# 14chanwa/remotesensingProject

Measured on AMD Instinct MI355X. Metric: Mpixel*disparity-hypotheses/s, higher is better.
Workload: dtype f32

## Files before the change

remotesensingproject_amd/build.py:

```python
from __future__ import annotations

import os
import re
import subprocess
import sys

HERE = os.path.dirname(os.path.abspath(__file__))
CSRC = os.path.join(HERE, "csrc")
OBJ = os.path.join(CSRC, "build")
SO = os.path.join(CSRC, "librslf_hip.so")
INCLUDE = os.path.join(os.path.dirname(HERE), "include")
COMMON = ["rslf_internal.hpp", "rslf_plan.hpp", "rslf_scratch.hpp", "rslf_device.hpp", "k2_taps.hpp", os.path.join(INCLUDE, "rslf_hip.h")]
UNITS = {
    "rslf_core.hip": ["k0_pack.hpp"],
    "rslf_pile.hip": ["k1_edge.hpp", "k_compact.hpp", "k2_scan.hpp", "k2_reg.hpp", "k2_stream.hpp", "k3_median.hpp"],
    "rslf_chip_a.hip": ["k2_scan.hpp", "k2_chip.hpp"],
    "rslf_chip_b.hip": ["k2_scan.hpp", "k2_chip.hpp"],
    "rslf_chip_c.hip": ["k2_scan.hpp", "k2_chip.hpp"],
    "rslf_scores.hip": ["k2_scan.hpp", "k2_reg.hpp", "k2_scores.hpp"],
    "rslf_peaks.hip": ["k8_peaks.hpp", "k8_peak_rule.hpp", "rslf_plan_peaks.hpp"],
    "rslf_subgrid.hip": ["k2_scan.hpp", "k9_subgrid.hpp", "k8_peak_rule.hpp", "rslf_plan_subgrid.hpp"],
    "rslf_sweep.hip": ["k3_median.hpp", "k4_propagate.hpp", "k_compact.hpp", "k2_scan.hpp", "k7_line_conf.hpp", "rslf_plan_subgrid.hpp",
                       "rslf_plan_sweep_peaks.hpp", "rslf_plan_peaks.hpp", "rslf_plan_sweep_gate.hpp", "k11_f2c_peak_rule.hpp"],
    "rslf_sweep_peaks.hip": ["k2_scan.hpp", "k10_sweep_peaks.hpp", "k10_peak_merge.hpp", "k8_peak_rule.hpp", "rslf_plan_sweep_peaks.hpp",
                             "rslf_plan_peaks.hpp", "rslf_plan_subgrid.hpp"],
    "rslf_f2c.hip": ["k5_f2c.hpp", "rslf_plan_f2c_peaks.hpp", "rslf_plan_peaks.hpp", "rslf_plan_f2c_consistency.hpp",
                     "rslf_plan_consistency.hpp", "k12_consistency_rule.hpp", "rslf_plan_derivative.hpp", "k17_derivative_rule.hpp"],
    "rslf_f2c_keep.hip": ["rslf_plan_f2c_peaks.hpp", "rslf_plan_peaks.hpp", "rslf_plan_sweep_gate.hpp", "k11_f2c_peak_rule.hpp",
                          "rslf_plan_f2c_consistency.hpp", "rslf_plan_consistency.hpp", "k12_consistency_rule.hpp"],
    "rslf_f2c_peaks.hip": ["k11_f2c_peaks.hpp", "k11_f2c_peak_rule.hpp", "rslf_plan_f2c_peaks.hpp", "rslf_plan_peaks.hpp"],
    "rslf_render.hip": ["k6_render.hpp", "rslf_plan_render.hpp"],
    "rslf_consistency.hip": ["k12_consistency.hpp", "k12_consistency_rule.hpp", "rslf_plan_consistency.hpp", "k13_f2c_consistency.hpp",
                             "rslf_plan_f2c_consistency.hpp"],
    "rslf_warp.hip": ["k14_view_warp.hpp", "k14_warp_rule.hpp", "rslf_plan_warp.hpp", "k12_consistency_rule.hpp"],
    "rslf_novel.hip": ["k15_novel_view.hpp", "k15_novel_rule.hpp", "rslf_plan_novel.hpp", "k14_warp_rule.hpp", "rslf_plan_warp.hpp",
                       "k12_consistency_rule.hpp"],
    "rslf_dilate.hip": ["k16_dilate.hpp", "k16_dilate_rule.hpp", "rslf_plan_dilate.hpp"],
    "rslf_derivative.hip": ["k17_derivative.hpp", "k17_derivative_rule.hpp", "rslf_plan_derivative.hpp"],
    "rslf_multi.hip": [],
    "rslf_multi_sweep.hip": [],
}
SOURCES = list(UNITS)

HIPCC_FLAGS = [
    "--offload-arch=gfx950",
# ... 131 lines not shown
```

remotesensingproject_amd/csrc/k2_reg.hpp:

```cpp
#pragma once

#include "k2_scan.hpp"
#include "k2_taps.hpp"

namespace rslf {

#ifndef RSLF_REG_GB104
#define RSLF_REG_GB104 8
#endif
constexpr int gather_batch(int c) { return c == 1 ? 8 : 4; }
constexpr int kPadSlack = 16;

template <int SPAD, int C, bool PK, bool KONLY>
__device__ __forceinline__ void mean_shift_pass(const float (&R)[PK ? 1 : C][PK ? 1 : SPAD], const f2 (&R2)[PK ? C : 1][PK ? SPAD / 2 : 1],
                                                int S, float kq, const float (&rbar)[C], float (&A)[C], float& B)
{
    static_assert(!KONLY || (C == 1 && !PK), "the K-only pass is written for the scalar one-channel blocks");
    if constexpr (PK) {
        f2 rb2[C];
        const f2 kq2 = {kq, kq};
#pragma unroll
        for (int c = 0; c < C; c++)
            rb2[c] = f2{rbar[c], rbar[c]};
        constexpr int kBlk = (C == 1) ? 8 : 4;
#pragma unroll
        for (int s0 = 0; s0 < SPAD; s0 += kBlk) {
            if (!(s0 < SPAD - kPadSlack || s0 < S))
                continue;
            if constexpr (C == 1) {
                f2 P[4], K[4];
                const f2 r4[4] = {R2[0][s0 / 2], R2[0][s0 / 2 + 1], R2[0][s0 / 2 + 2], R2[0][s0 / 2 + 3]};
                mean_shift_pk_octet(r4, rb2[0], kq2, P, K);
#pragma unroll
                for (int j = 0; j < 4; j++) {
                    A[0] = A[0] + P[j].x;
                    B = B + K[j].x;
                    A[0] = A[0] + P[j].y;
                    B = B + K[j].y;
                }
            } else {
                f2 Pa[3], Pb[3], Ka, Kb;
                const f2 ra[3] = {R2[0][s0 / 2], R2[1][s0 / 2], R2[C - 1][s0 / 2]};
                const f2 rb[3] = {R2[0][s0 / 2 + 1], R2[1][s0 / 2 + 1], R2[C - 1][s0 / 2 + 1]};
                const f2 m[3] = {rb2[0], rb2[C > 1 ? 1 : 0], rb2[C - 1]};
                mean_shift_pk_rgb_quad(ra, rb, m, kq2, Pa, Pb, Ka, Kb);
#pragma unroll
                for (int c = 0; c < C; c++)
                    A[c] = A[c] + Pa[c].x;
                B = B + Ka.x;
#pragma unroll
                for (int c = 0; c < C; c++)
                    A[c] = A[c] + Pa[c].y;
                B = B + Ka.y;
#pragma unroll
                for (int c = 0; c < C; c++)
                    A[c] = A[c] + Pb[c].x;
                B = B + Kb.x;
#pragma unroll
                for (int c = 0; c < C; c++)
                    A[c] = A[c] + Pb[c].y;
                B = B + Kb.y;
            }
        }
    } else if (C == 1) {
#pragma unroll
        for (int s0 = 0; s0 < SPAD; s0 += 4) {
            if (s0 + 4 <= SPAD - kPadSlack || s0 + 4 <= S) {
                if constexpr (KONLY)
                    mean_shift_group4_k(R[0][s0], R[0][s0 + 1], R[0][s0 + 2], R[0][s0 + 3], rbar[0], kq, B);
                else
                    mean_shift_group4(R[0][s0], R[0][s0 + 1], R[0][s0 + 2], R[0][s0 + 3], rbar[0], kq, A[0], B);
            } else {
#pragma unroll
                for (int j = 0; j < 3; j++)
                    if (s0 + j < S) {
                        if constexpr (KONLY)
                            mean_shift_group1_k(R[0][s0 + j], rbar[0], kq, B);
                        else
                            mean_shift_group1(R[0][s0 + j], rbar[0], kq, A[0], B);
                    }
            }
        }
    } else {
#pragma unroll
        for (int s = 0; s < SPAD; s++) {
            if (!(s < SPAD - kPadSlack || s < S))
                continue;
            float q[C];
#pragma unroll
            for (int c = 0; c < C; c++) {
                const float delta = R[c][s] - rbar[c];
                const float tq = kq * delta;
                q[c] = tq * delta;
            }
            float qs = q[0];
            if (C == 3) {
                qs = q[0] + q[C - 1];
                qs = qs + q[C > 1 ? 1 : 0];
            }
            const float K = kernel_weight(qs);
#pragma unroll
            for (int c = 0; c < C; c++) {
                const float pr = R[c][s] * K;
                A[c] = A[c] + pr;
            }
            B = B + K;
        }
    }
}

template <int SPAD, int C, int BATCH>
__device__ __forceinline__ void tap_table_batch(const float* epi, const float* otab, const int* tboff, const f2* tw, unsigned du_bytes,
                                                float uf, int S, int stride_s, bool from_table, int g, int& rowoff, float (&R)[C][SPAD])
{
// ... 27 lines not shown
    }
    rowoff += BATCH * stride_s;
#pragma unroll
    for (int j = 0; j < BATCH; j++) {
        const int s = g * BATCH + j;
#pragma unroll
        for (int c = 0; c < C; c++) {
            e0[c][j] = kSentinel;
            e1[c][j] = 0.0f;
        }
        if (s < SPAD - kPadSlack || s < S) {
            const float* p = (const float*)((const char*)epi + bo[j]);
#pragma unroll
            for (int c = 0; c < C; c++) {
                e0[c][j] = p[c];
                e1[c][j] = p[C + c];
            }
        }
    }
#pragma unroll
    for (int j = 0; j < BATCH; j++) {
        const int s = g * BATCH + j;
#pragma unroll
        for (int c = 0; c < C; c++) {
            const float m0 = om[j] * e0[c][j];
            const float m1 = tt[j] * e1[c][j];
            const float r = m0 + m1;
            R[c][s] = (s < SPAD - kPadSlack || s < S) ? r : kSentinel;
        }
    }
}

template <int SPAD, int C, bool BORDER, bool UNIFORM_D, bool PK, int GB = 0, class BestT = Best<C>, bool LANE_D = false,
          bool TRIM = false, bool TAPS = false>
__device__ __forceinline__ void scan_reg_body(const ScanArgs& a, int v, int u, int d0, int d1, BestT& best,
                                              float* __restrict__ otab, int dlane = 0, int dstep = 1)
{
    static_assert(!LANE_D || !UNIFORM_D, "hypotheses in the lanes: every lane has its own view offsets");
    constexpr int kGatherBatch = GB > 0 ? GB : (C == 1 && !PK && SPAD == 104 && RSLF_REG_GB104 == 13) ? 13 : gather_batch(C);
    static_assert(SPAD % kGatherBatch == 0 && (!PK || kGatherBatch % 2 == 0), "whole batches, whole pairs");
    static_assert(SPAD % 8 == 0, "slot counts are multiples of 8");
    static_assert(!TAPS || (UNIFORM_D && !BORDER && !PK), "the tap table belongs to the interior scalar uniform-D row form");
    const VolView& vol = a.vol;
    const float* epi = vol.row(v, 0);
    const float uf = (float)u;
    const int Um1 = vol.U - 1;
    const unsigned Um1_bits = __float_as_uint((float)Um1);
    const int S = vol.S;
    const int lane = threadIdx.x & 63;
    const long long o = (long long)v * vol.U + u;
    const float dmin = a.dmin_vu ? a.dmin_vu[o] : a.dmin;
    const float dmax = a.dmax_vu ? a.dmax_vu[o] : a.dmax;
    const float range = dmax - dmin;
    const float denom = (float)(a.dim_d - 1);
    const float kq = (C == 1) ? a.k.k1 : a.k.inv_h2;
    const float slope = a.k.slope;
    const int stride_s = (int)vol.stride_s;
    float centre[C];
#pragma unroll
    for (int c = 0; c < C; c++)
        centre[c] = epi[(long long)a.s_hat * vol.stride_s + u * C + c];
    int* const tboff = TAPS ? reinterpret_cast<int*>(otab + SPAD) : nullptr;
    f2* const tw = TAPS ? reinterpret_cast<f2*>(otab + 2 * SPAD) : nullptr;
    int u_first = 0, u_last = 0;
    unsigned du_bytes = 0;
    bool taps_on = false;
    if constexpr (TAPS) {
        u_first = __builtin_amdgcn_readfirstlane(u);
        u_last = __builtin_amdgcn_readlane(u, 63);
        const int du = u - u_first;
        du_bytes = (unsigned)(du * C) << 2;
        taps_on = a.tap_table != 0 && __all(du == min(lane, u_last - u_first));
    }

#pragma unroll 1
    for (int dk = d0; dk < d1; dk += (LANE_D ? dstep : 1)) {
        const int d = LANE_D ? min(dk + dlane, d1 - 1) : dk;
        const float Dd = hypothesis(dmin, range, denom, d);
        float R[PK ? 1 : C][PK ? 1 : SPAD];
        f2 R2[PK ? C : 1][PK ? SPAD / 2 : 1];
        int card = BORDER ? 0 : S;
        float Ss0 = (float)a.s_hat;
        asm volatile("" : "+v"(Ss0));
        int rowoff = 0;
        asm volatile("" : "+s"(rowoff));
        unsigned fastb = 0;
        if (UNIFORM_D) {
            int lane_s = lane, tile_first = u_first, tile_last = u_last;
            if constexpr (TAPS)
                asm volatile("" : "+v"(lane_s), "+s"(tile_first), "+s"(tile_last));
#pragma unroll
            for (int s0 = 0; s0 < SPAD; s0 += 64) {
                const int s = s0 + lane_s;
                float off = (float)(a.s_hat - s) * Dd;
                off = off * slope;
                if (SPAD % 64 == 0 || s < SPAD)
                    otab[s] = off;
                if constexpr (TAPS) {
                    if (taps_on) {
                        const TapEntry e = tap_entry(off, tile_first, tile_last, vol.U, C, __mul24(s, stride_s));
                        if (SPAD % 64 == 0 || s < SPAD) {
                            tboff[s] = e.byteoff;
                            tw[s] = f2{e.t, e.omt};
                        }
                        unsigned long long m = __ballot(e.fast);
                        m &= m >> 1;
                        m &= m >> 2;
                        m &= m >> 4;
                        static_assert(!TAPS || kGatherBatch == 8, "the batch bits are gathered for batches of eight samples");
#pragma unroll
                        for (int k = 0; k < 8; k++)
                            if (s0 + 8 * k < SPAD)
                                fastb |= ((unsigned)(m >> (8 * k)) & 1u) << (s0 / 8 + k);
                    }
                }
            }
            __builtin_amdgcn_wave_barrier();
            if constexpr (TAPS)
                fastb = __builtin_amdgcn_readfirstlane(fastb & (S >= SPAD ? ~0u : (1u << (S / kGatherBatch)) - 1u));
        }
#pragma unroll
        for (int g = 0; g < SPAD / kGatherBatch; g++) {
            if constexpr (TAPS) {
                tap_table_batch<SPAD, C, kGatherBatch>(epi, otab, tboff, tw, du_bytes, uf, S, stride_s, (fastb >> g) & 1u, g, rowoff, R);
            } else {
                float tt[kGatherBatch], e0[C][kGatherBatch], e1[C][kGatherBatch];
                bool ok[kGatherBatch];
#pragma unroll
                for (int j = 0; j < kGatherBatch; j++) {
                    const int s = g * kGatherBatch + j;
                    tt[j] = 0.0f;
                    ok[j] = false;
#pragma unroll
                    for (int c = 0; c < C; c++) {
                        e0[c][j] = kSentinel;
                        e1[c][j] = 0.0f;
                    }
                    if (s < SPAD - kPadSlack || s < S) {
                        float x;
                        if (UNIFORM_D) {
                            x = otab[s];
                        } else {
                            x = (Ss0 - (float)s) * Dd;
                            x = x * slope;
                        }
                        x = x + uf;
                        tt[j] = lerp_weight(x);
                        int i0 = floor_to_int(x);
                        ok[j] = true;
                        if (BORDER) {
                            ok[j] = __float_as_uint(x) <= Um1_bits;
                            i0 = ok[j] ? i0 : 0;
                        }
                        const unsigned byteoff = (unsigned)(i0 * C + rowoff) << 2;
                        const float* p = (const float*)((const char*)epi + byteoff);
// ... 22 lines not shown
                        if constexpr (PK) {
                            if (s & 1)
                                R2[c][s >> 1].y = val;
                            else
                                R2[c][s >> 1].x = val;
                        } else {
                            R[c][s] = val;
                        }
                    }
                    if (BORDER)
                        card += ok[j] ? 1 : 0;
                }
            }
            {
                const int b = g * kGatherBatch;
#pragma unroll
                for (int c = 0; c < C; c++) {
                    if constexpr (PK) {
                        asm volatile("" : "+v"(R2[c][b / 2]), "+v"(R2[c][b / 2 + 1]));
                        if (kGatherBatch == 8)
                            asm volatile("" : "+v"(R2[c][b / 2 + 2]), "+v"(R2[c][b / 2 + 3]));
                        static_assert(!PK || kGatherBatch == 4 || kGatherBatch == 8, "pair pinning is written for 4 and 8");
                    } else if (kGatherBatch != 4 && kGatherBatch != 8) {
#pragma unroll
                        for (int j = 0; j < kGatherBatch; j++)
                            asm volatile("" : "+v"(R[c][b + j]));
                    } else {
                        asm volatile("" : "+v"(R[c][b + 0]), "+v"(R[c][b + 1]), "+v"(R[c][b + 2]), "+v"(R[c][b + 3]));
                        if (kGatherBatch == 8)
                            asm volatile("" : "+v"(R[c][b + kGatherBatch - 4]), "+v"(R[c][b + kGatherBatch - 3]),
                                              "+v"(R[c][b + kGatherBatch - 2]), "+v"(R[c][b + kGatherBatch - 1]));
                    }
                }
                if (BORDER)
                    asm volatile("" : "+s"(rowoff), "+v"(Ss0), "+v"(card));
                else
                    asm volatile("" : "+s"(rowoff), "+v"(Ss0));
            }
        }

        float rbar[C];
#pragma unroll
        for (int c = 0; c < C; c++)
            rbar[c] = centre[c];
        float B = 0.0f;
#pragma unroll 1
        for (int it = 0; it < a.k.n_iter; it++) {
            float A[C];
#pragma unroll
            for (int c = 0; c < C; c++)
                A[c] = 0.0f;
            B = 0.0f;
            if constexpr (TRIM) {
                if (it == a.k.n_iter - 1) {
                    mean_shift_pass<SPAD, C, PK, true>(R, R2, S, kq, rbar, A, B);
                    break;
                }
            }
            mean_shift_pass<SPAD, C, PK, false>(R, R2, S, kq, rbar, A, B);
#pragma unroll
            for (int c = 0; c < C; c++) {
                const float qd = (B != 0.0f) ? (A[c] / B) : 0.0f;
                rbar[c] = (qd > 0.0f) ? qd : 0.0f;
            }
        }
        const float cardf = (float)card;
        float sc = (card != 0) ? (B / cardf) : 0.0f;
        sc = (sc > 0.0f) ? sc : 0.0f;
        if (!LANE_D || dk + dlane < d1)
            best.offer(sc, d, Dd, rbar);
    }
}

template <int C>
struct LastPassRbar {
    __device__ __forceinline__ void operator()(const ScanArgs& a, long long o, float Dd, float (&rbar)[C]) const
    {
        if (a.k.n_iter == 0)
            return;
        const VolView& vol = a.vol;
        const int v = (int)(o / vol.U);
        const int u = (int)(o - (long long)v * vol.U);
        const float* epi = vol.row(v, 0);
        const float uf = (float)u;
        const unsigned Um1_bits = __float_as_uint((float)(vol.U - 1));
        const float kq = (C == 1) ? a.k.k1 : a.k.inv_h2;
        const float Ss0 = (float)a.s_hat;
        const int S = vol.S;
        float A[C];
#pragma unroll
        for (int c = 0; c < C; c++)
            A[c] = 0.0f;
// ... 156 lines not shown
                const float m0 = w[j].y * e0[j];
                const float m1 = w[j].x * e1[j];
                R[0][g * BATCH + j] = m0 + m1;
            }
#pragma unroll
            for (int j = 0; j < BATCH; j++)
                asm volatile("" : "+v"(R[0][g * BATCH + j]));
#pragma unroll
            for (int j = 0; j < BATCH; j++)
                cur[j] = nxt[j];
        }

        float rbar[C] = {centre};
        float B = 0.0f;
#pragma unroll 1
        for (int it = 0; it < a.k.n_iter; it++) {
            float A[C] = {0.0f};
            B = 0.0f;
            if (it == a.k.n_iter - 1) {
                mean_shift_pass<SPAD, C, false, true>(R, R2, S, kq, rbar, A, B);
                break;
            }
            mean_shift_pass<SPAD, C, false, false>(R, R2, S, kq, rbar, A, B);
            const float qd = (B != 0.0f) ? (A[0] / B) : 0.0f;
            rbar[0] = (qd > 0.0f) ? qd : 0.0f;
        }
        const float cardf = (float)S;
        float sc = (S != 0) ? (B / cardf) : 0.0f;
        sc = (sc > 0.0f) ? sc : 0.0f;
        best.offer(sc, d, Dd, rbar);
    }
}

template <int SPAD, int C>
using ScanRegRbarFix = std::conditional_t<scan_reg_trim(SPAD, C), LastPassRbar<C>, NoRbarFix>;

template <int SPAD, int C, class BestT>
__device__ __forceinline__ void scan_reg_rows(const ScanArgs& a, int v, int u, int d0, int d1, BestT& best, float* otab)
{
    constexpr bool PK = scan_reg_packed_math(SPAD, C);
    constexpr bool kTaps = scan_reg_tap_table(SPAD, C);
    if (a.dmin_vu) {
        scan_reg_body<SPAD, C, true, false, PK, 0, BestT, false, scan_reg_trim(SPAD, C)>(a, v, u, d0, d1, best, otab);
        return;
    }
    const float max_ds = (float)max(a.s_hat, a.vol.S - 1 - a.s_hat);
    const float range = a.dmax - a.dmin, denom = (float)(a.dim_d - 1);
    const float uf = (float)u, Um1 = (float)(a.vol.U - 1);
    if constexpr (scan_reg_scalar_taps(SPAD, C)) {
        typedef const __attribute__((address_space(4))) float* FloatPtr;
        typedef const __attribute__((address_space(4))) int* IntPtr;
        const bool rx = a.rx_off != nullptr;
        auto form = [&](int d) -> int {
            const float Dd = rx ? ((FloatPtr)a.rx_D)[d] : hypothesis(a.dmin, range, denom, d);
            const float reach = max_ds * fabsf(Dd) * fabsf(a.k.slope) + 2.0f;
            const bool in = __all((uf - reach >= 0.0f) && (uf + reach <= Um1));
            return !in ? 0 : (rx && ((IntPtr)a.rx_exact)[d]) ? 2 : 1;
        };
        int d = d0;
        while (d < d1) {
            const int f = form(d);
            int e = d + 1;
            while (e < d1 && form(e) == f)
                e++;
            if (f == 2)
                scan_reg_body_scalar<SPAD>(a, v, u, d, e, best);
            else if (f == 1)
                scan_reg_body<SPAD, C, false, true, PK, 0, BestT, false, scan_reg_trim(SPAD, C), kTaps>(a, v, u, d, e, best, otab);
            else
                scan_reg_body<SPAD, C, true, true, PK, 0, BestT, false, scan_reg_trim(SPAD, C)>(a, v, u, d, e, best, otab);
            d = e;
        }
        return;
    }
    auto interior = [&](int d) -> bool {
        const float reach = max_ds * fabsf(hypothesis(a.dmin, range, denom, d)) * fabsf(a.k.slope) + 2.0f;
        return __all((uf - reach >= 0.0f) && (uf + reach <= Um1));
    };
    int d = d0;
    while (d < d1) {
        const bool in = interior(d);
        int e = d + 1;
        while (e < d1 && interior(e) == in)
            e++;
        if (in)
            scan_reg_body<SPAD, C, false, true, PK, 0, BestT, false, scan_reg_trim(SPAD, C), kTaps>(a, v, u, d, e, best, otab);
        else
            scan_reg_body<SPAD, C, true, true, PK, 0, BestT, false, scan_reg_trim(SPAD, C)>(a, v, u, d, e, best, otab);
        d = e;
    }
}

template <int SPAD, int C>
__global__ __launch_bounds__(64 * kScanWaves) __attribute__((amdgpu_waves_per_eu(scan_reg_waves(SPAD, C), scan_reg_waves(SPAD, C))))
void k2_scan_reg(ScanArgs a)
{
    __shared__ __attribute__((aligned(16))) float s_otab[kScanWaves][SPAD * (scan_reg_tap_table(SPAD, C) ? 4 : 1)];
    float* otab = s_otab[__builtin_amdgcn_readfirstlane(threadIdx.x >> 6)];
    constexpr bool kEpiDyn = false;
    float* const epi_lds = nullptr;
    const int epi_stride = 0;
    using Fix = ScanRegRbarFix<SPAD, C>;
    if constexpr (scan_reg_best_in_lds(SPAD, C)) {
        __shared__ float s_best[kScanWaves][BestLds<C>::kFloats];
        BestLds<C> running(s_best[__builtin_amdgcn_readfirstlane(threadIdx.x >> 6)]);
        RSLF_SCAN_ROW_TILE_FIX((running.init(), scan_reg_rows<SPAD, C>(a, v, u, d0, d1, running, otab), running.load(best)), Fix{})
    } else {
        RSLF_SCAN_ROW_TILE_FIX((scan_reg_rows<SPAD, C>(a, v, u, d0, d1, best, otab)), Fix{})
    }
}

#ifndef RSLF_PACKED_LONG_GB
#define RSLF_PACKED_LONG_GB 4
#endif
constexpr bool packed_long_unit(int spad, int c) { return c == 1 && spad >= 80 && spad <= 128 && spad % RSLF_PACKED_LONG_GB == 0; }
constexpr int packed_waves(int spad, int c) { return packed_long_unit(spad, c) ? 2 : scan_reg_waves(spad + 24, c); }
constexpr int packed_gather_batch(int spad, int c) { return packed_long_unit(spad, c) ? spad / RSLF_PACKED_LONG_GB : 0; }

template <int SPAD, int C>
__global__ __launch_bounds__(64 * kScanWaves) __attribute__((amdgpu_waves_per_eu(packed_waves(SPAD, C), packed_waves(SPAD, C))))
void k2_scan_reg_packed(ScanArgs a)
// ... 48 lines not shown
```

remotesensingproject_amd/csrc/k2_scan.hpp:

```cpp
#pragma once

#include <type_traits>

#include "rslf_device.hpp"

namespace rslf {

constexpr int kScanWaves = 4;
#ifndef RSLF_XCD_ROW_INTERLEAVE
#define RSLF_XCD_ROW_INTERLEAVE 1
#endif

struct ScanArgs {
    VolView vol;
    const int* list;
    const int* count;
    const float* dmin_vu;
    const float* dmax_vu;
    float dmin, dmax;
    int dim_d, s_hat;
    ScanConsts k;
    float* Ce;
    uint8_t* Ce_mask;
    float* Cd;
    float* depth;
    float* rbar;
    int32_t* idx;
    float* score;
    int tile_w;
    int tiles_per_row;
    int logical_blocks;
    int per_xcd;
    int groups;
    struct Partial* partial;
    int* ticket;
    int v0;
    int packed;
    const int* packed_n;
    int packed_adapt;
    int stream_park;
    int stream_wave_floats;
    float stream_frac_max;
    int px_waves;
    const int* rowbase;
    int row_min;
    int tap_table;
    const long long* rx_off;
    const float* rx_w;
    const float* rx_D;
    const int* rx_exact;
};


struct Partial {
    float score, D;
    int d;
    float rbar[3];
    double sum;
};

template <int C>
struct Best {
    float score;
    int d;
    float D;
    float rbar[C];
    double sum;
    __device__ __forceinline__ void init()
    {
        score = -1.0f;
        d = 0;
        D = 0.0f;
#pragma unroll
        for (int c = 0; c < C; c++)
            rbar[c] = 0.0f;
        sum = 0.0;
    }
    __device__ __forceinline__ void offer(float sc, int dd, float Dd, const float (&rb)[C])
    {
// ... 545 lines not shown
```

remotesensingproject_amd/csrc/k2_scores.hpp:

```cpp
#pragma once

#include "k2_reg.hpp"
#include "rslf_plan.hpp"

namespace rslf {

constexpr int kScoreRun = plan::kScoreRun;
constexpr int kScorePitch = kScoreRun + 1;
static_assert(64 % kScoreRun == 0, "a store instruction covers whole runs");

struct ScoreDst {
    float* scores;
    int v_first;
};

template <int C>
struct ScoreRows {
    float* park;
    const int* pix;
    float* row;
    int dim_d, d_lo, d_hi;
    __device__ __forceinline__ ScoreRows(float* park_, int* pix_, const ScanArgs& a, const ScoreDst& dst, int v, int u, bool active,
                                         int d0, int d1)
        : park(park_), pix(pix_), row(dst.scores + (size_t)(v - dst.v_first) * (size_t)a.vol.U * (size_t)a.dim_d), dim_d(a.dim_d),
// ... 6 lines not shown
        const int k = (d - d_lo) % kScoreRun;
        park[(threadIdx.x & 63) * kScorePitch + k] = sc;
        if (k == kScoreRun - 1 || d == d_hi - 1)
            flush(d - k, k + 1);
    }
    __device__ __forceinline__ void flush(int d_first, int n)
    {
        __builtin_amdgcn_fence(__ATOMIC_RELEASE, "wavefront");
        __builtin_amdgcn_wave_barrier();
        const int lane = threadIdx.x & 63;
        const int j = lane % kScoreRun, q = lane / kScoreRun;
#pragma unroll 4
        for (int p0 = 0; p0 < 64; p0 += 64 / kScoreRun) {
            const int p = p0 + q;
            const float sc = park[p * kScorePitch + j];
            const int u = pix[p];
            if (j < n && u >= 0)
                row[(size_t)u * (size_t)dim_d + (size_t)(d_first + j)] = sc;
        }
        __builtin_amdgcn_wave_barrier();
        __builtin_amdgcn_fence(__ATOMIC_ACQUIRE, "wavefront");
    }
};

constexpr bool score_rows_trim(int spad, int c) { return c == 1 && !scan_reg_packed_math(spad, c); }
constexpr bool score_rows_tap_table(int spad, int c) { return scan_reg_tap_table(spad, c) && score_rows_trim(spad, c); }

template <int SPAD, int C>
__device__ __forceinline__ void score_reg_rows(const ScanArgs& a, int v, int u, int d0, int d1, ScoreRows<C>& rows, float* otab)
{
    constexpr bool PK = scan_reg_packed_math(SPAD, C);
    constexpr bool kTrim = score_rows_trim(SPAD, C);
    constexpr bool kTaps = score_rows_tap_table(SPAD, C);
    if (a.dmin_vu) {
        scan_reg_body<SPAD, C, true, false, PK, 0, ScoreRows<C>, false, kTrim>(a, v, u, d0, d1, rows, otab);
        return;
    }
    const float max_ds = (float)max(a.s_hat, a.vol.S - 1 - a.s_hat);
    const float range = a.dmax - a.dmin, denom = (float)(a.dim_d - 1);
    const float uf = (float)u, Um1 = (float)(a.vol.U - 1);
    auto interior = [&](int d) -> bool {
        const float reach = max_ds * fabsf(hypothesis(a.dmin, range, denom, d)) * fabsf(a.k.slope) + 2.0f;
        return __all((uf - reach >= 0.0f) && (uf + reach <= Um1));
    };
    int d = d0;
    while (d < d1) {
        const bool in = interior(d);
        int e = d + 1;
        while (e < d1 && interior(e) == in)
            e++;
        if (in)
            scan_reg_body<SPAD, C, false, true, PK, 0, ScoreRows<C>, false, kTrim, kTaps>(a, v, u, d, e, rows, otab);
        else
            scan_reg_body<SPAD, C, true, true, PK, 0, ScoreRows<C>, false, kTrim>(a, v, u, d, e, rows, otab);
        d = e;
    }
}

#define RSLF_SCORE_ROW_TILE(SCAN_CALL)                                                                                     \
    __shared__ float s_park[kScanWaves][64 * kScorePitch];                                                                 \
    __shared__ int s_pix[kScanWaves][64];                                                                                  \
    int v, u, d0, d1;                                                                                                      \
    bool active;                                                                                                           \
    const int lb = RSLF_XCD_ROW_INTERLEAVE ? xcd_logical_block_rows(blockIdx.x, a.tiles_per_row * a.groups)                \
                                           : xcd_logical_block(blockIdx.x, a.per_xcd);                                     \
    if (!scan_tile(a, lb, v, u, active))                                                                                   \
        return;                                                                                                            \
    scan_chunk(a, lb % a.groups, d0, d1);                                                                                  \
    const int wave = __builtin_amdgcn_readfirstlane(threadIdx.x >> 6);                                                     \
    ScoreRows<C> rows(s_park[wave], s_pix[wave], a, dst, v, u, active, d0, d1);                                            \
    SCAN_CALL;

template <int SPAD, int C>
__global__ __launch_bounds__(64 * kScanWaves) __attribute__((amdgpu_waves_per_eu(scan_reg_waves(SPAD, C), scan_reg_waves(SPAD, C))))
void k2_score_rows_reg(ScanArgs a, ScoreDst dst)
{
    constexpr int kTable = score_rows_tap_table(SPAD, C) ? 4 : 1;
    __shared__ __attribute__((aligned(16))) float s_otab[kScanWaves][SPAD * kTable];
    static_assert(sizeof(float) * kScanWaves * (64 * kScorePitch + 64 + SPAD * kTable) == plan::score_lds_bytes(SPAD, kTable) &&
                      plan::score_lds_bytes(SPAD, kTable) <= plan::kScoreLdsLimit, "rslf_plan.hpp states this kernel's LDS");
    float* otab = s_otab[__builtin_amdgcn_readfirstlane(threadIdx.x >> 6)];
    RSLF_SCORE_ROW_TILE((score_reg_rows<SPAD, C>(a, v, u, d0, d1, rows, otab)))
}

template <int C>
__global__ __launch_bounds__(64 * kScanWaves) void k2_score_rows_generic(ScanArgs a, ScoreDst dst)
{
// ... 44 lines not shown
```

remotesensingproject_amd/csrc/rslf_core.hip:

```cpp
#include "rslf_internal.hpp"

#include <algorithm>
#include <cmath>

#include "k0_pack.hpp"

using namespace rslf;


namespace rslf {

char* last_error_buffer()
{
    static thread_local char g_err[512] = "";
    return g_err;
}

static std::atomic<int> g_inject[kInjectSites];

bool inject_hit(InjectSite site)
{
    std::atomic<int>& c = g_inject[site];
    int v = c.load(std::memory_order_relaxed);
    while (v > 0)
// ... 186 lines not shown
    return RSLF_OK;
}
RSLF_API_CATCH

extern "C" int rslf_ctx_set_stream(rslf_ctx* ctx, void* hip_stream) RSLF_API_TRY
{
    if (!ctx)
        return fail(RSLF_ERR_INVALID_ARG, "ctx is NULL");
    ctx->stream = (hipStream_t)hip_stream;
    return RSLF_OK;
}
RSLF_API_CATCH

extern "C" int rslf_ctx_set_debug(rslf_ctx* ctx, const char* key, int value) RSLF_API_TRY
{
    if (!ctx || !key)
        return fail(RSLF_ERR_INVALID_ARG, "ctx/key is NULL");
    if (strcmp(key, "force_scan") == 0 && value >= 0 && value <= 2)
        ctx->force_scan = value;
    else if (strcmp(key, "force_groups") == 0 && value >= 0 && value <= 64)
        ctx->force_groups = value;
    else if (strcmp(key, "force_packed") == 0 && value >= -1 && value <= 1)
        ctx->force_packed = value;
    else if (strcmp(key, "px") == 0 && value >= -1 && value <= 1)
        ctx->px_mode = value;
    else if (strcmp(key, "stream_share") == 0 && value >= 0 && value <= 2)
        ctx->stream_share = value;
    else if (strcmp(key, "row_split") == 0 && value >= 0 && value <= 65536)
        ctx->row_split = value;
    else if (strcmp(key, "tap_table") == 0 && (value == 0 || value == 1))
        ctx->tap_table = value;
    else if (strcmp(key, "scalar_taps") == 0 && (value == 0 || value == 1))
        ctx->scalar_taps = value;
    else if (strcmp(key, "claim_skip") == 0 && (value == 0 || value == 1))
        ctx->claim_skip = value;
    else if (strcmp(key, "subgrid_list") == 0 && (value == 0 || value == 1))
        ctx->subgrid_list = value;
    else if (strcmp(key, "peaks_list") == 0 && (value == 0 || value == 1))
        ctx->peaks_list = value;
    else if (strcmp(key, "consistency_order") == 0 && value >= 0 && value <= 2)
        ctx->consistency_order = value;
    else if (strcmp(key, "time_all") == 0 && (value == 0 || value == 1)) {
        ctx->time_all = value;
        ctx->ev_used = 0;
    } else if (strcmp(key, "stream_groups") == 0 && value >= 0 && value <= 64)
        ctx->stream_groups = value;
    else if (strcmp(key, "stream_lds_kib") == 0 && value >= 16 && value <= 152) {
        ctx->stream_lds_bytes = (size_t)value << 10;
    } else if (strcmp(key, "staging_kib") == 0 && value >= 0 && value <= 262144)
        ctx->staging_kib = value;
    else
        return fail(RSLF_ERR_INVALID_ARG, "rslf_ctx_set_debug: unknown key or value out of range: %s = %d", key, value);
    return RSLF_OK;
}
RSLF_API_CATCH

extern "C" int rslf_ctx_synchronize(rslf_ctx* ctx) RSLF_API_TRY
{
    if (!ctx)
        return fail(RSLF_ERR_INVALID_ARG, "ctx is NULL");
    HIP_TRY(hipSetDevice(ctx->device));
    HIP_TRY(hipStreamSynchronize(ctx->stream));
    return RSLF_OK;
}
RSLF_API_CATCH

// ... 500 lines not shown
```

remotesensingproject_amd/csrc/rslf_internal.hpp:

```cpp
#pragma once

#include "../../include/rslf_hip.h"

#include <hip/hip_runtime.h>

#include <atomic>
#include <cstdarg>
#include <cstdio>
#include <cstring>
#include <exception>
#include <functional>
#include <memory>
#include <new>
#include <string>
#include <thread>
#include <vector>

#include "rslf_device.hpp"
#include "rslf_plan.hpp"
#include "rslf_scratch.hpp"


namespace rslf {

// ... 191 lines not shown
    bool subgrid = false;
    bool peaks = false;
    rslf_peaks pk = {};
    int dim_d = 0;
    float prop_ratio = 0.0f;
};

}

struct rslf_ctx {
    int device = 0;
    hipStream_t stream = nullptr;
    rslf::Scratch scratch;
    rslf::SweepState sweep;
    hipEvent_t ev0 = nullptr, ev1 = nullptr;
    bool ev_valid = false;
    int time_all = 0;
    std::vector<hipEvent_t> ev_pool;
    size_t ev_used = 0;
    int last_spad = 0;
    int last_kernel = 0;
    bool last_gated = false;
    int num_cus = 0;
    int force_scan = 0;
    int force_groups = 0;
    int force_packed = -1;
    int px_mode = -1;
    int stream_groups = 0;
    int stream_share = 1;
    size_t stream_lds_bytes = rslf::plan::kStreamLdsBytes;
    int row_split = 1;
    int tap_table = 1;
    int scalar_taps = 1;
    rslf::RowExactKey row_exact_key;
    bool last_row_exact = false;
    int subgrid_list = 1;
    int peaks_list = 1;
    int claim_skip = 1;
    int staging_kib = 0;
    int consistency_order = 0;
};

struct rslf_volume {
    rslf_ctx* ctx = nullptr;
    int device = 0;
    int V = 0, S = 0, U = 0, C = 0, pitch = 0;
    float* base = nullptr;
    size_t bytes = 0;
    float min_value = 0.0f, max_value = 0.0f;
    bool filled = false;
};

struct rslf_multi {
    struct Dev {
        rslf_ctx* ctx = nullptr;
        hipStream_t s_up = nullptr, s_comp = nullptr, s_down = nullptr;
        hipEvent_t done[2] = {nullptr, nullptr};
        rslf_volume* vol[2] = {nullptr, nullptr};
        rslf::DeviceBuf planes[2];
        rslf::PinnedBuf pin[2];
        rslf::DeviceBuf arena;
    };
    std::vector<Dev> devs;
    int chunk_rows = 0;
    std::vector<unsigned char> peer;
};
// ... 226 lines not shown
```

remotesensingproject_amd/csrc/rslf_pile.hip:

```cpp
#include "rslf_internal.hpp"

#include <algorithm>
#include <cmath>

#include "k1_edge.hpp"
#include "k2_scan.hpp"
#include "k2_reg.hpp"
#include "k2_stream.hpp"
#include "k3_median.hpp"

using namespace rslf;

static_assert(sizeof(Partial) == plan::kPartialRecordBytes, "rslf_plan.hpp sizes the record scratch");
static_assert(kScanWaves == plan::kScanWavesPerTile, "rslf_plan.hpp shares the hypotheses out over this many waves");
static_assert(!RSLF_SCALAR_TAPS || !RSLF_TAP_TABLE || (scan_reg_scalar_taps(104, 1) && row_exact_slots(104, 1) == 104),
              "rslf_internal.hpp names the kernel that has the scalar-tap form");


extern "C" int rslf_edge_confidence_pile(rslf_ctx* ctx, const rslf_volume* vol, int s, const rslf_params* p,
                                         float* d_Ce_vu, uint8_t* d_Ce_mask_vu) RSLF_API_TRY
{
    if (!ctx || !vol || !d_Ce_vu || !d_Ce_mask_vu)
        return fail(RSLF_ERR_INVALID_ARG, "NULL argument");
    int rc = check_params(p);
// ... 279 lines not shown
    if (r.err) {
        ctx->row_exact_key = RowExactKey{};
        HIP_TRY(hip_err(r));
    }
    char* base = ctx->scratch.row_exact.as<char>();
    long long* d_off = reinterpret_cast<long long*>(base);
    f2* d_w = reinterpret_cast<f2*>(d_off + (size_t)a.dim_d * slots);
    float* d_D = reinterpret_cast<float*>(d_w + (size_t)a.dim_d * slots);
    int* d_exact = reinterpret_cast<int*>(d_D + a.dim_d);
    if (r.fresh || !key.same(ctx->row_exact_key)) {
        ctx->row_exact_key = RowExactKey{};
        hipLaunchKernelGGL(k2_fill_row_exact, dim3(a.dim_d), dim3(128), 0, st, a.dmin, a.dmax, a.dim_d, a.k.slope, a.s_hat, a.vol.S, slots,
                           a.vol.U, a.vol.C, (int)a.vol.stride_s, d_off, d_w, d_D, d_exact);
        HIP_TRY(hipGetLastError());
        ctx->row_exact_key = key;
    }
    a.rx_off = d_off;
    a.rx_w = reinterpret_cast<const float*>(d_w);
    a.rx_D = d_D;
    a.rx_exact = d_exact;
    ctx->last_row_exact = true;
    return RSLF_OK;
}

static void apply_plan(ScanArgs& a, const plan::ScanPlan& p, const rslf_ctx* ctx)
{
    a.groups = p.groups;
    a.tile_w = p.tile_w;
    a.tiles_per_row = p.tiles_per_row;
    a.packed = p.packed ? 1 : 0;
    a.packed_adapt = p.packed_adapt ? 1 : 0;
    a.px_waves = p.px_waves;
    a.tap_table = p.tap_table;
    a.stream_park = p.stream_park;
    a.stream_wave_floats = p.stream_wave_floats;
    a.partial = p.groups > 1 ? ctx->scratch.scan_partial.as<Partial>() : nullptr;
    a.ticket = p.groups > 1 ? ctx->scratch.scan_ticket.as<int>() : nullptr;
}

static int enqueue_scan(const plan::ScanPlan& p, const ScanArgs& a, unsigned grid_x, size_t stream_lds_bytes, hipStream_t st)
{
    const dim3 grid(grid_x), block(64 * kScanWaves);
    const int C = a.vol.C;
    hipError_t attr = hipSuccess;
    auto stream = [&](auto kernel) {
        attr = hipFuncSetAttribute(reinterpret_cast<const void*>(kernel), hipFuncAttributeMaxDynamicSharedMemorySize, (int)stream_lds_bytes);
        if (attr == hipSuccess)
            hipLaunchKernelGGL(kernel, grid, block, p.lds_bytes, st, a);
    };
    int rc = RSLF_OK;
    switch (p.kind) {
    case RSLF_SCAN_REG:
    case RSLF_SCAN_REG_PX:
        rc = launch_scan_reg(p.spad, C, a, grid, st);
        break;
    case RSLF_SCAN_CHIP:
        rc = launch_scan_chip(a, grid, p.lds_bytes, st);
        break;
    case RSLF_SCAN_STREAM_PX:
        if (C == 1)
            stream_px_kernel_for<1>(p.stream_nres, stream);
        else
            stream_px_kernel_for<3>(p.stream_nres, stream);
        break;
    case RSLF_SCAN_STREAM:
        if (p.packed && C == 1)
// ... 517 lines not shown
```

remotesensingproject_amd/csrc/rslf_scores.hip:

```cpp
#include "rslf_internal.hpp"

#include <algorithm>

#include "k2_scores.hpp"

using namespace rslf;

static_assert(kScanWaves == plan::kScanWavesPerTile, "rslf_plan.hpp shares the hypotheses out over this many waves");

static int launch_score_rows_reg(int spad, int C, const ScanArgs& a, const ScoreDst& dst, dim3 grid, hipStream_t stream)
{
#define RSLF_CASE(N)                                                                                              \
    case N:                                                                                                       \
        hipLaunchKernelGGL((k2_score_rows_reg<N, RSLF_C>), grid, dim3(64 * kScanWaves), 0, stream, a, dst);       \
        return RSLF_OK;
    if (C == 1) {
        switch (spad) {
#define RSLF_C 1
            RSLF_SPAD_LIST_1CH(RSLF_CASE)
#undef RSLF_C
        default:
            break;
        }
    } else if (C == 3) {
// ... 43 lines not shown
    const int kind = plan::choose_score_kernel(vol->S, vol->C, plan::scan_range_ok(vol->min_value, vol->max_value),
                                               p->interpolation == RSLF_INTERP_LINEAR, ctx->force_scan, &spad);
    const plan::ScanPlan sp = plan::score_plan(kind, spad, n_rows, vol->U, dim_d, ctx->num_cus, spad ? scan_reg_waves(spad, vol->C) : 4,
                                               ctx->force_groups);
    std::vector<plan::ScanLaunch> launches;
    long long tiles = 0;
    if (!plan::score_launches(v_first, n_rows, vol->U, sp, &launches, &tiles))
        return fail(RSLF_ERR_UNSUPPORTED, "%lld tiles x %d groups exceeds the grid limit", tiles, sp.groups);

    hipStream_t st = ctx->stream;
    const Scratch& sc = ctx->scratch;
    int* const list = own ? own->list : sc.list.as<int>();
    int* const count = own ? own->count : sc.count.as<int>();
    unsigned long long* const total = own ? own->total : sc.pixel_total();
    HIP_TRY(hipMemsetAsync(total, 0, sizeof(unsigned long long), st));
    hipLaunchKernelGGL(k_score_lists, dim3(n_rows), dim3(256), 0, st, d_mask_vu, vol->U, v_first, list, count, total);
    HIP_TRY(hipGetLastError());

    ScanArgs a = {};
    a.vol = view_of(vol);
    a.list = list;
    a.count = count;
    a.dmin_vu = d_dmin_vu;
    a.dmax_vu = d_dmax_vu;
    a.dmin = dmin;
    a.dmax = dmax;
    a.dim_d = dim_d;
    a.s_hat = s_hat;
    a.k = make_scan_consts(p);
    a.groups = sp.groups;
    a.tile_w = sp.tile_w;
    a.tiles_per_row = sp.tiles_per_row;
    a.tap_table = spad ? ctx->tap_table : 0;
    const ScoreDst dst = {d_scores, v_first};
    for (const plan::ScanLaunch& l : launches) {
        a.v0 = l.v0, a.logical_blocks = l.logical_blocks, a.per_xcd = l.per_xcd;
        if (kind == RSLF_SCAN_REG) {
            rc = launch_score_rows_reg(spad, vol->C, a, dst, dim3(l.grid), st);
            if (rc)
                return rc;
        } else if (vol->C == 1) {
            hipLaunchKernelGGL(k2_score_rows_generic<1>, dim3(l.grid), dim3(64 * kScanWaves), 0, st, a, dst);
        } else {
            hipLaunchKernelGGL(k2_score_rows_generic<3>, dim3(l.grid), dim3(64 * kScanWaves), 0, st, a, dst);
        }
        HIP_TRY(hipGetLastError());
    }
    *kind_out = kind;
    *spad_out = spad;
    return RSLF_OK;
}

void rslf::score_stats(unsigned long long pixels, int dim_d, int kind, int spad, rslf_stats* stats)
{
    stats->pixels_scanned = (int64_t)pixels;
    stats->units = (int64_t)pixels * dim_d;
    stats->scan_kernel = kind;
    stats->s_pad = spad;
}

int rslf::read_pixel_total(rslf_ctx* ctx, unsigned long long* tot)
{
    HIP_TRY(hipMemcpyAsync(tot, ctx->scratch.pixel_total(), sizeof(*tot), hipMemcpyDeviceToHost, ctx->stream));
    HIP_TRY(hipStreamSynchronize(ctx->stream));
    return RSLF_OK;
}
// ... 71 lines not shown
```

remotesensingproject_amd/depth.py:

```python
from __future__ import annotations

import atexit
import copy
import ctypes as C
import sys
from dataclasses import dataclass
from typing import NamedTuple, Optional, Sequence

import numpy as np
import torch

from . import _lib
from ._lib import RslfParams, RslfStats, RslfVolumeDesc, check


class Interpolation1DLinear:
    mode = 0


class Interpolation1DNearestNeighbour:

    def __init__(self, as_built: bool = False):
        self.mode = 2 if as_built else 1

# ... 117 lines not shown
        w = float(derivative_channels)
    except (TypeError, ValueError):
        w = float("nan")
    if isinstance(derivative_channels, bool) or not np.isfinite(w) or w <= 0 or w > float(np.finfo(np.float32).max):
        raise ValueError("%s: derivative_channels %r is not 0 (off) or a finite weight > 0" % (who, derivative_channels))
    return w


def require_no_derivative_channels(derivative_channels, who: str) -> None:
    if derivative_channels is not None and derivative_channels is not False and derivative_channels != 0:
        raise ValueError("%s: derivative_channels=%r is not built here (one device: fine_to_coarse_run_host, FineToCoarse; or "
                         "Volume.with_derivative_channels)" % (who, derivative_channels))


class Context:

    def __init__(self, device: int | torch.device | None = None):
        if device is None:
            device = torch.cuda.current_device()
        self.device = torch.device("cuda", device) if isinstance(device, int) else torch.device(device)
        h = C.c_void_p()
        check(_lib.lib().rslf_ctx_create(self.device.index or 0, C.byref(h)), "rslf_ctx_create")
        self._h = h
        self.use_current_stream()

    def use_current_stream(self) -> None:
        s = torch.cuda.current_stream(self.device).cuda_stream
        check(_lib.lib().rslf_ctx_set_stream(self._h, C.c_void_p(s)), "rslf_ctx_set_stream")

    def synchronize(self) -> None:
        check(_lib.lib().rslf_ctx_synchronize(self._h), "rslf_ctx_synchronize")

    _DEBUG_DEFAULTS = dict(force_scan=0, force_groups=0, force_packed=-1, px=-1, stream_share=1, stream_groups=0, stream_lds_kib=80,
                           claim_skip=1, time_all=0, row_split=1, staging_kib=0, tap_table=1, scalar_taps=1,
                           subgrid_list=1, peaks_list=1, consistency_order=0)
    _FORCE_SCAN = {None: 0, "auto": 0, "generic": 1, "stream": 2}

    def set_debug(self, **hooks) -> None:
        for k, v in hooks.items():
            if k == "force_scan" and not isinstance(v, int):
                v = self._FORCE_SCAN[v or None]
            check(_lib.lib().rslf_ctx_set_debug(self._h, k.encode(), int(v)), "rslf_ctx_set_debug(%s)" % k)

    def reset_debug(self) -> None:
        self.set_debug(**self._DEBUG_DEFAULTS)

    def last_scan_kernel_ms(self) -> float:
        ms = C.c_float()
        check(_lib.lib().rslf_last_scan_kernel_ms(self._h, C.byref(ms)), "rslf_last_scan_kernel_ms")
        return float(ms.value)

    def last_scan_row_exact(self) -> tuple[bool, int]:
        a, n = C.c_int(), C.c_int()
        check(_lib.lib().rslf_last_scan_row_exact(self._h, C.byref(a), C.byref(n)), "rslf_last_scan_row_exact")
        return bool(a.value), int(n.value)

    def scan_time_total_ms(self) -> tuple[float, int]:
        ms, n = C.c_float(), C.c_int()
        check(_lib.lib().rslf_scan_time_total_ms(self._h, C.byref(ms), C.byref(n)), "rslf_scan_time_total_ms")
        return float(ms.value), int(n.value)

    def get_withheld_sources(self) -> int:
        n = C.c_ulonglong()
        check(_lib.lib().rslf_sweep_withheld(self._h, C.byref(n)), "rslf_sweep_withheld")
        return int(n.value)

    def close(self) -> None:
# ... 1953 lines not shown
```

Before: 8365.

## Skip gathers and mean-shift passes for views dead across a border tile

In the border form of the scalar one-channel TRIM register scan, each view offset is tested against the tile's u range; views whose sample positions fall entirely outside the image for the whole wave are marked dead via a ballot, and the contiguous live span is turned into a unit mask. Gather batches and mean-shift pass groups outside the live span are skipped, cutting loads and ALU work on border tiles. This adds ballot and mask-building overhead and wave-uniform branches in an otherwise fully unrolled loop, which may affect register allocation and scheduling.

```diff
diff --git a/remotesensingproject_amd/build.py b/remotesensingproject_amd/build.py
--- a/remotesensingproject_amd/build.py
+++ b/remotesensingproject_amd/build.py
@@ -10,7 +10,7 @@
 OBJ = os.path.join(CSRC, "build")
 SO = os.path.join(CSRC, "librslf_hip.so")
 INCLUDE = os.path.join(os.path.dirname(HERE), "include")
-COMMON = ["rslf_internal.hpp", "rslf_plan.hpp", "rslf_scratch.hpp", "rslf_device.hpp", "k2_taps.hpp", os.path.join(INCLUDE, "rslf_hip.h")]
+COMMON = ["rslf_internal.hpp", "rslf_plan.hpp", "rslf_scratch.hpp", "rslf_device.hpp", "k2_taps.hpp", "k2_live.hpp", os.path.join(INCLUDE, "rslf_hip.h")]
 UNITS = {
     "rslf_core.hip": ["k0_pack.hpp"],
     "rslf_pile.hip": ["k1_edge.hpp", "k_compact.hpp", "k2_scan.hpp", "k2_reg.hpp", "k2_stream.hpp", "k3_median.hpp"],
diff --git a/remotesensingproject_amd/csrc/k2_live.hpp b/remotesensingproject_amd/csrc/k2_live.hpp
--- /dev/null
+++ b/remotesensingproject_amd/csrc/k2_live.hpp
@@ -0,0 +1,66 @@
+#pragma once
+
+#include <stdint.h>
+#include <string.h>
+
+#if defined(__HIPCC__)
+#define RSLF_LIVE_FN __host__ __device__ __forceinline__
+#else
+#define RSLF_LIVE_FN inline
+#endif
+
+namespace rslf {
+
+RSLF_LIVE_FN bool view_dead(float off, float u_min_f, float u_max_f, float Um1_f)
+{
+    const float x_max = off + u_max_f;
+    const float x_min = off + u_min_f;
+    return x_max < 0.0f || x_min > Um1_f;
+}
+
+RSLF_LIVE_FN bool sample_valid(float off, float u_f, float Um1_f)
+{
+    const float x = off + u_f;
+    uint32_t xb, ub;
+#if defined(__HIP_DEVICE_COMPILE__)
+    xb = __float_as_uint(x), ub = __float_as_uint(Um1_f);
+#else
+    memcpy(&xb, &x, sizeof(xb));
+    memcpy(&ub, &Um1_f, sizeof(ub));
+#endif
+    return xb <= ub;
+}
+
+struct LiveSpan {
+    int lo, hi;
+};
+template <int WORDS>
+RSLF_LIVE_FN LiveSpan live_span(const unsigned long long (&bits)[WORDS], int spad, int S)
+{
+    LiveSpan r = {spad, 0};
+#if defined(__HIPCC__)
+#pragma unroll
+#endif
+    for (int w = 0; w < WORDS; w++) {
+        const unsigned long long m = bits[w];
+        if (m) {
+            const int first = w * 64 + __builtin_ctzll(m);
+            const int last = w * 64 + 63 - __builtin_clzll(m);
+            r.lo = first < r.lo ? first : r.lo;
+            r.hi = last + 1 > r.hi ? last + 1 : r.hi;
+        }
+    }
+    r.hi = S < r.hi ? S : r.hi;
+    return r;
+}
+
+RSLF_LIVE_FN unsigned long long live_units(LiveSpan sp, int width)
+{
+    if (sp.hi <= sp.lo)
+        return 0ull;
+    const int k_lo = sp.lo / width, k_hi = (sp.hi + width - 1) / width;
+    const unsigned long long below_hi = k_hi >= 64 ? ~0ull : (1ull << k_hi) - 1ull;
+    return below_hi & ~((1ull << k_lo) - 1ull);
+}
+
+}
diff --git a/remotesensingproject_amd/csrc/k2_reg.hpp b/remotesensingproject_amd/csrc/k2_reg.hpp
--- a/remotesensingproject_amd/csrc/k2_reg.hpp
+++ b/remotesensingproject_amd/csrc/k2_reg.hpp
@@ -1,6 +1,7 @@
 #pragma once
 
 #include "k2_scan.hpp"
+#include "k2_live.hpp"
 #include "k2_taps.hpp"
 
 namespace rslf {
@@ -11,11 +12,24 @@
 constexpr int gather_batch(int c) { return c == 1 ? 8 : 4; }
 constexpr int kPadSlack = 16;
 
-template <int SPAD, int C, bool PK, bool KONLY>
+template <int SPAD>
+using LiveMask = std::conditional_t<(SPAD / 4 <= 32), unsigned, unsigned long long>;
+#ifndef RSLF_LIVE_UNIT
+#define RSLF_LIVE_UNIT 8
+#endif
+static_assert(RSLF_LIVE_UNIT % 4 == 0 && RSLF_LIVE_UNIT >= 4 && RSLF_LIVE_UNIT <= 32, "whole groups of four");
+template <int SPAD>
+__device__ __forceinline__ bool live_unit(LiveMask<SPAD> live4, int u0, int width)
+{
+    return ((live4 >> (u0 / 4)) & ((LiveMask<SPAD>(1) << (width / 4)) - 1)) != 0;
+}
+template <int SPAD, int C, bool PK, bool KONLY, bool LIVE = false>
 __device__ __forceinline__ void mean_shift_pass(const float (&R)[PK ? 1 : C][PK ? 1 : SPAD], const f2 (&R2)[PK ? C : 1][PK ? SPAD / 2 : 1],
-                                                int S, float kq, const float (&rbar)[C], float (&A)[C], float& B)
+                                                int S, float kq, const float (&rbar)[C], float (&A)[C], float& B,
+                                                LiveMask<SPAD> live4 = 0)
 {
     static_assert(!KONLY || (C == 1 && !PK), "the K-only pass is written for the scalar one-channel blocks");
+    static_assert(!LIVE || (C == 1 && !PK), "live views are skipped in the scalar one-channel blocks");
     if constexpr (PK) {
         f2 rb2[C];
         const f2 kq2 = {kq, kq};
@@ -63,8 +77,15 @@
             }
         }
     } else if (C == 1) {
-#pragma unroll
-        for (int s0 = 0; s0 < SPAD; s0 += 4) {
+        if constexpr (LIVE)
+            asm volatile("" : "+s"(live4));
+        constexpr int kUnit = LIVE ? RSLF_LIVE_UNIT : 4;
+#pragma unroll
+        for (int u0 = 0; u0 < SPAD; u0 += kUnit) {
+            if (LIVE && !__builtin_expect(live_unit<SPAD>(live4, u0, kUnit), 1))
+                continue;
+#pragma unroll
+        for (int s0 = u0; s0 < (u0 + kUnit < SPAD ? u0 + kUnit : SPAD); s0 += 4) {
             if (s0 + 4 <= SPAD - kPadSlack || s0 + 4 <= S) {
                 if constexpr (KONLY)
                     mean_shift_group4_k(R[0][s0], R[0][s0 + 1], R[0][s0 + 2], R[0][s0 + 3], rbar[0], kq, B);
@@ -80,6 +101,7 @@
                             mean_shift_group1(R[0][s0 + j], rbar[0], kq, A[0], B);
                     }
             }
+        }
         }
     } else {
 #pragma unroll
@@ -173,14 +195,16 @@
 }
 
 template <int SPAD, int C, bool BORDER, bool UNIFORM_D, bool PK, int GB = 0, class BestT = Best<C>, bool LANE_D = false,
-          bool TRIM = false, bool TAPS = false>
+          bool TRIM = false, bool TAPS = false, bool LIVE = false>
 __device__ __forceinline__ void scan_reg_body(const ScanArgs& a, int v, int u, int d0, int d1, BestT& best,
                                               float* __restrict__ otab, int dlane = 0, int dstep = 1)
 {
     static_assert(!LANE_D || !UNIFORM_D, "hypotheses in the lanes: every lane has its own view offsets");
+    static_assert(!LIVE || (BORDER && UNIFORM_D && TRIM && C == 1 && !PK && !TAPS), "live views: the border form of the scalar one-channel TRIM row kernels");
     constexpr int kGatherBatch = GB > 0 ? GB : (C == 1 && !PK && SPAD == 104 && RSLF_REG_GB104 == 13) ? 13 : gather_batch(C);
     static_assert(SPAD % kGatherBatch == 0 && (!PK || kGatherBatch % 2 == 0), "whole batches, whole pairs");
     static_assert(SPAD % 8 == 0, "slot counts are multiples of 8");
+    static_assert(!LIVE || kGatherBatch % 4 == 0, "a pass group of four lies within one gather batch: gathered whole or not at all");
     static_assert(!TAPS || (UNIFORM_D && !BORDER && !PK), "the tap table belongs to the interior scalar uniform-D row form");
     const VolView& vol = a.vol;
     const float* epi = vol.row(v, 0);
@@ -226,7 +250,15 @@
         int rowoff = 0;
         asm volatile("" : "+s"(rowoff));
         unsigned fastb = 0;
+        unsigned long long live_bits[(SPAD + 63) / 64] = {};
         if (UNIFORM_D) {
+            float u_min_f = 0.0f, u_max_f = 0.0f;
+            if constexpr (LIVE) {
+                int u_tile = u;
+                asm volatile("" : "+v"(u_tile));
+                u_min_f = a.live_views ? (float)__builtin_amdgcn_readfirstlane(u_tile) : -INFINITY;
+                u_max_f = a.live_views ? (float)__builtin_amdgcn_readlane(u_tile, 63) : INFINITY;
+            }
             int lane_s = lane, tile_first = u_first, tile_last = u_last;
             if constexpr (TAPS)
                 asm volatile("" : "+v"(lane_s), "+s"(tile_first), "+s"(tile_last));
@@ -237,6 +269,8 @@
                 off = off * slope;
                 if (SPAD % 64 == 0 || s < SPAD)
                     otab[s] = off;
+                if constexpr (LIVE)
+                    live_bits[s0 / 64] = __ballot(!view_dead(off, u_min_f, u_max_f, (float)Um1));
                 if constexpr (TAPS) {
                     if (taps_on) {
                         const TapEntry e = tap_entry(off, tile_first, tile_last, vol.U, C, __mul24(s, stride_s));
@@ -260,8 +294,18 @@
             if constexpr (TAPS)
                 fastb = __builtin_amdgcn_readfirstlane(fastb & (S >= SPAD ? ~0u : (1u << (S / kGatherBatch)) - 1u));
         }
+        LiveMask<SPAD> live4 = 0;
+        if constexpr (LIVE)
+            live4 = (LiveMask<SPAD>)live_units(live_span(live_bits, SPAD, S), 4);
+        constexpr int kLiveUnit = RSLF_LIVE_UNIT > kGatherBatch ? RSLF_LIVE_UNIT : kGatherBatch;
+        static_assert(!LIVE || (kLiveUnit % kGatherBatch == 0 && kLiveUnit % RSLF_LIVE_UNIT == 0), "units of whole batches and whole pass units");
 #pragma unroll
         for (int g = 0; g < SPAD / kGatherBatch; g++) {
+            if (!LIVE || __builtin_expect(live_unit<SPAD>(live4, g * kGatherBatch / kLiveUnit * kLiveUnit, kLiveUnit), 1)) {
+            if constexpr (LIVE) {
+                rowoff = g * kGatherBatch * stride_s;
+                asm volatile("" : "+s"(rowoff));
+            }
             if constexpr (TAPS) {
                 tap_table_batch<SPAD, C, kGatherBatch>(epi, otab, tboff, tw, du_bytes, uf, S, stride_s, (fastb >> g) & 1u, g, rowoff, R);
             } else {
@@ -350,11 +394,14 @@
                                               "+v"(R[c][b + kGatherBatch - 2]), "+v"(R[c][b + kGatherBatch - 1]));
                     }
                 }
-                if (BORDER)
-                    asm volatile("" : "+s"(rowoff), "+v"(Ss0), "+v"(card));
-                else
-                    asm volatile("" : "+s"(rowoff), "+v"(Ss0));
-            }
+            }
+            }
+            if constexpr (LIVE)
+                asm volatile("" : "+v"(card));
+            else if (BORDER)
+                asm volatile("" : "+s"(rowoff), "+v"(Ss0), "+v"(card));
+            else
+                asm volatile("" : "+s"(rowoff), "+v"(Ss0));
         }
 
         float rbar[C];
@@ -371,11 +418,11 @@
             B = 0.0f;
             if constexpr (TRIM) {
                 if (it == a.k.n_iter - 1) {
-                    mean_shift_pass<SPAD, C, PK, true>(R, R2, S, kq, rbar, A, B);
+                    mean_shift_pass<SPAD, C, PK, true, LIVE>(R, R2, S, kq, rbar, A, B, live4);
                     break;
                 }
             }
-            mean_shift_pass<SPAD, C, PK, false>(R, R2, S, kq, rbar, A, B);
+            mean_shift_pass<SPAD, C, PK, false, LIVE>(R, R2, S, kq, rbar, A, B, live4);
 #pragma unroll
             for (int c = 0; c < C; c++) {
                 const float qd = (B != 0.0f) ? (A[c] / B) : 0.0f;
@@ -598,6 +645,11 @@
     }
 }
 
+#ifndef RSLF_LIVE_VIEWS
+#define RSLF_LIVE_VIEWS 1
+#endif
+constexpr bool scan_reg_live_views(int spad, int c) { return RSLF_LIVE_VIEWS && scan_reg_trim(spad, c); }
+
 template <int SPAD, int C>
 using ScanRegRbarFix = std::conditional_t<scan_reg_trim(SPAD, C), LastPassRbar<C>, NoRbarFix>;
 
@@ -606,6 +658,7 @@
 {
     constexpr bool PK = scan_reg_packed_math(SPAD, C);
     constexpr bool kTaps = scan_reg_tap_table(SPAD, C);
+    constexpr bool kLive = scan_reg_live_views(SPAD, C);
     if (a.dmin_vu) {
         scan_reg_body<SPAD, C, true, false, PK, 0, BestT, false, scan_reg_trim(SPAD, C)>(a, v, u, d0, d1, best, otab);
         return;
@@ -634,7 +687,7 @@
             else if (f == 1)
                 scan_reg_body<SPAD, C, false, true, PK, 0, BestT, false, scan_reg_trim(SPAD, C), kTaps>(a, v, u, d, e, best, otab);
             else
-                scan_reg_body<SPAD, C, true, true, PK, 0, BestT, false, scan_reg_trim(SPAD, C)>(a, v, u, d, e, best, otab);
+                scan_reg_body<SPAD, C, true, true, PK, 0, BestT, false, scan_reg_trim(SPAD, C), false, kLive>(a, v, u, d, e, best, otab);
             d = e;
         }
         return;
@@ -652,7 +705,7 @@
         if (in)
             scan_reg_body<SPAD, C, false, true, PK, 0, BestT, false, scan_reg_trim(SPAD, C), kTaps>(a, v, u, d, e, best, otab);
         else
-            scan_reg_body<SPAD, C, true, true, PK, 0, BestT, false, scan_reg_trim(SPAD, C)>(a, v, u, d, e, best, otab);
+            scan_reg_body<SPAD, C, true, true, PK, 0, BestT, false, scan_reg_trim(SPAD, C), false, kLive>(a, v, u, d, e, best, otab);
         d = e;
     }
 }
diff --git a/remotesensingproject_amd/csrc/k2_scan.hpp b/remotesensingproject_amd/csrc/k2_scan.hpp
--- a/remotesensingproject_amd/csrc/k2_scan.hpp
+++ b/remotesensingproject_amd/csrc/k2_scan.hpp
@@ -45,6 +45,7 @@
     const int* rowbase;
     int row_min;
     int tap_table;
+    int live_views;
     const long long* rx_off;
     const float* rx_w;
     const float* rx_D;
diff --git a/remotesensingproject_amd/csrc/k2_scores.hpp b/remotesensingproject_amd/csrc/k2_scores.hpp
--- a/remotesensingproject_amd/csrc/k2_scores.hpp
+++ b/remotesensingproject_amd/csrc/k2_scores.hpp
@@ -62,6 +62,7 @@
     constexpr bool PK = scan_reg_packed_math(SPAD, C);
     constexpr bool kTrim = score_rows_trim(SPAD, C);
     constexpr bool kTaps = score_rows_tap_table(SPAD, C);
+    constexpr bool kLive = scan_reg_live_views(SPAD, C) && kTrim;
     if (a.dmin_vu) {
         scan_reg_body<SPAD, C, true, false, PK, 0, ScoreRows<C>, false, kTrim>(a, v, u, d0, d1, rows, otab);
         return;
@@ -82,7 +83,7 @@
         if (in)
             scan_reg_body<SPAD, C, false, true, PK, 0, ScoreRows<C>, false, kTrim, kTaps>(a, v, u, d, e, rows, otab);
         else
-            scan_reg_body<SPAD, C, true, true, PK, 0, ScoreRows<C>, false, kTrim>(a, v, u, d, e, rows, otab);
+            scan_reg_body<SPAD, C, true, true, PK, 0, ScoreRows<C>, false, kTrim, false, kLive>(a, v, u, d, e, rows, otab);
         d = e;
     }
 }
diff --git a/remotesensingproject_amd/csrc/rslf_core.hip b/remotesensingproject_amd/csrc/rslf_core.hip
--- a/remotesensingproject_amd/csrc/rslf_core.hip
+++ b/remotesensingproject_amd/csrc/rslf_core.hip
@@ -242,6 +242,8 @@
         ctx->tap_table = value;
     else if (strcmp(key, "scalar_taps") == 0 && (value == 0 || value == 1))
         ctx->scalar_taps = value;
+    else if (strcmp(key, "live_views") == 0 && (value == 0 || value == 1))
+        ctx->live_views = value;
     else if (strcmp(key, "claim_skip") == 0 && (value == 0 || value == 1))
         ctx->claim_skip = value;
     else if (strcmp(key, "subgrid_list") == 0 && (value == 0 || value == 1))
diff --git a/remotesensingproject_amd/csrc/rslf_internal.hpp b/remotesensingproject_amd/csrc/rslf_internal.hpp
--- a/remotesensingproject_amd/csrc/rslf_internal.hpp
+++ b/remotesensingproject_amd/csrc/rslf_internal.hpp
@@ -247,6 +247,7 @@
     int row_split = 1;
     int tap_table = 1;
     int scalar_taps = 1;
+    int live_views = 1;
     rslf::RowExactKey row_exact_key;
     bool last_row_exact = false;
     int subgrid_list = 1;
diff --git a/remotesensingproject_amd/csrc/rslf_pile.hip b/remotesensingproject_amd/csrc/rslf_pile.hip
--- a/remotesensingproject_amd/csrc/rslf_pile.hip
+++ b/remotesensingproject_amd/csrc/rslf_pile.hip
@@ -335,6 +335,7 @@
     a.packed_adapt = p.packed_adapt ? 1 : 0;
     a.px_waves = p.px_waves;
     a.tap_table = p.tap_table;
+    a.live_views = ctx->live_views;
     a.stream_park = p.stream_park;
     a.stream_wave_floats = p.stream_wave_floats;
     a.partial = p.groups > 1 ? ctx->scratch.scan_partial.as<Partial>() : nullptr;
diff --git a/remotesensingproject_amd/csrc/rslf_scores.hip b/remotesensingproject_amd/csrc/rslf_scores.hip
--- a/remotesensingproject_amd/csrc/rslf_scores.hip
+++ b/remotesensingproject_amd/csrc/rslf_scores.hip
@@ -99,6 +99,7 @@
     a.tile_w = sp.tile_w;
     a.tiles_per_row = sp.tiles_per_row;
     a.tap_table = spad ? ctx->tap_table : 0;
+    a.live_views = ctx->live_views;
     const ScoreDst dst = {d_scores, v_first};
     for (const plan::ScanLaunch& l : launches) {
         a.v0 = l.v0, a.logical_blocks = l.logical_blocks, a.per_xcd = l.per_xcd;
diff --git a/remotesensingproject_amd/depth.py b/remotesensingproject_amd/depth.py
--- a/remotesensingproject_amd/depth.py
+++ b/remotesensingproject_amd/depth.py
@@ -173,7 +173,7 @@
         check(_lib.lib().rslf_ctx_synchronize(self._h), "rslf_ctx_synchronize")
 
     _DEBUG_DEFAULTS = dict(force_scan=0, force_groups=0, force_packed=-1, px=-1, stream_share=1, stream_groups=0, stream_lds_kib=80,
-                           claim_skip=1, time_all=0, row_split=1, staging_kib=0, tap_table=1, scalar_taps=1,
+                           claim_skip=1, time_all=0, row_split=1, staging_kib=0, tap_table=1, scalar_taps=1, live_views=1,
                            subgrid_list=1, peaks_list=1, consistency_order=0)
     _FORCE_SCAN = {None: 0, "auto": 0, "generic": 1, "stream": 2}
 
```

New measurement: 8421 (median of 6 runs). No clear change (+0.7%).
